# AdamClixby/Modulate

Measured on NVIDIA B200. Metric: ark_dtb_decrypt_throughput, higher is better.
Workload: dtype u8

## Files before the change

### modulate_b200/csrc/cycle_kernels.cu

```cuda
#include "cycle_kernels.cuh"
#include "lcg.h"

#include <cstdlib>

namespace modk {

using modlcg::mulmod;
using modlcg::step_lazy;
using modlcg::low8_canonical;

#ifndef MODK_CANON_FMA_MASK
#define MODK_CANON_FMA_MASK 0x5
#endif
#ifndef MODK_MIN_CTAS
#define MODK_MIN_CTAS 10
#endif
#ifndef MODK_MIN_CTAS_INLINE
#define MODK_MIN_CTAS_INLINE 8
#endif
#ifndef MODK_MIN_CTAS_COAL
#define MODK_MIN_CTAS_COAL 10
#endif
#ifndef MODK_STAGE
#define MODK_STAGE 1
#endif
#ifndef MODK_EDGE_ROUNDS
#define MODK_EDGE_ROUNDS 1
#endif
#ifndef MODK_STAGE_SEQ
#define MODK_STAGE_SEQ 1
#endif
#ifndef MODK_GENERAL_FULL
#define MODK_GENERAL_FULL 1
#endif
#ifndef MODK_HOIST_POW
#define MODK_HOIST_POW 1
#endif
#ifndef MODK_REC_PREFETCH
#define MODK_REC_PREFETCH 2048
#endif

constexpr int kTw0Size = 1024;
constexpr int kTw1Size = (int)(((1ull << 32) / kTileBytes) / kTw0Size + 2);

__constant__ uint32_t c_tw0[kTw0Size];
__constant__ uint32_t c_tw1[kTw1Size];
__constant__ uint32_t c_ainv[16];
__device__ uint32_t g_chunk_pow2[kChunksPerTile];

__device__ __forceinline__ uint32_t jump_lazy(uint32_t st, uint32_t y2)
{
    const uint64_t p = (uint64_t)st * (uint64_t)y2;
    return (uint32_t)(p >> 32) + ((uint32_t)p >> 1);
}


__device__ __forceinline__ uint4 ldg128(uint64_t addr)
{
    uint4 r;
    asm volatile("ld.global.v4.u32 {%0, %1, %2, %3}, [%4];" : "=r"(r.x), "=r"(r.y), "=r"(r.z), "=r"(r.w) : "l"(addr));
    return r;
}

__device__ __forceinline__ void stg128(uint64_t addr, const uint4& v)
{
    asm volatile("st.global.v4.u32 [%0], {%1, %2, %3, %4};" ::"l"(addr), "r"(v.x), "r"(v.y), "r"(v.z), "r"(v.w));
}

#if MODK_STAGE

__device__ __forceinline__ uint32_t smem_u32(const void* p) { return (uint32_t)__cvta_generic_to_shared(p); }

__device__ __forceinline__ void mbar_init(uint32_t bar, uint32_t count)
{
    asm volatile("mbarrier.init.shared::cta.b64 [%0], %1;" ::"r"(bar), "r"(count));
    asm volatile("fence.mbarrier_init.release.cluster;" ::: "memory");
}

__device__ __forceinline__ void mbar_expect_tx(uint32_t bar, uint32_t bytes)
{
    asm volatile("mbarrier.arrive.expect_tx.shared::cta.b64 _, [%0], %1;" ::"r"(bar), "r"(bytes) : "memory");
}

__device__ __forceinline__ void mbar_wait(uint32_t bar, uint32_t parity)
{
    asm volatile(
        "{\n"
        ".reg .pred p;\n"
        "MODK_WAIT:\n"
        "mbarrier.try_wait.parity.shared::cta.b64 p, [%0], %1;\n"
        "@p bra MODK_DONE;\n"
        "bra MODK_WAIT;\n"
        "MODK_DONE:\n"
        "}\n" ::"r"(bar), "r"(parity) : "memory");
}

__device__ __forceinline__ void bulk_g2s(uint32_t dst_smem, uint64_t src_gmem, uint32_t bytes, uint32_t bar)
{
    asm volatile("cp.async.bulk.shared::cluster.global.mbarrier::complete_tx::bytes [%0], [%1], %2, [%3];" ::"r"(dst_smem),
                 "l"(src_gmem), "r"(bytes), "r"(bar)
                 : "memory");
}

__device__ __forceinline__ uint4 lds128(uint32_t addr)
{
    uint4 r;
    asm volatile("ld.shared.v4.u32 {%0, %1, %2, %3}, [%4];" : "=r"(r.x), "=r"(r.y), "=r"(r.z), "=r"(r.w) : "r"(addr));
    return r;
}
#endif


__device__ __forceinline__ uint32_t low8_canonical_fma(uint32_t s, uint32_t two)
{
    uint32_t r;
    asm("mad.hi.u32 %0, %1, %2, %1;" : "=r"(r) : "r"(s), "r"(two));
    return r;
}

__device__ __noinline__ uint4 cycle_chunk_exact(uint4 d, uint32_t s, const uint32_t two)
{
    uint32_t w[4] = {d.x, d.y, d.z, d.w};
#pragma unroll
    for (int j = 0; j < 4; ++j) {
        s = step_lazy(s);
        const uint32_t b0 = (MODK_CANON_FMA_MASK & 1) ? low8_canonical_fma(s, two) : low8_canonical(s);
        s = step_lazy(s);
        const uint32_t b1 = (MODK_CANON_FMA_MASK & 2) ? low8_canonical_fma(s, two) : low8_canonical(s);
        s = step_lazy(s);
        const uint32_t b2 = (MODK_CANON_FMA_MASK & 4) ? low8_canonical_fma(s, two) : low8_canonical(s);
        s = step_lazy(s);
        const uint32_t b3 = (MODK_CANON_FMA_MASK & 8) ? low8_canonical_fma(s, two) : low8_canonical(s);
        const uint32_t lo = __byte_perm(b0, b1, 0x0040);
        const uint32_t hi = __byte_perm(b2, b3, 0x0040);
        w[j] ^= __byte_perm(lo, hi, 0x5410);
    }
    return make_uint4(w[0], w[1], w[2], w[3]);
}


__device__ __noinline__ void store_partial(uint64_t addr, uint4 v, uint32_t lo, uint32_t hi)
{
    const uint32_t w[4] = {v.x, v.y, v.z, v.w};
#pragma unroll
    for (uint32_t k = 0; k < 4; ++k) {
        const uint32_t b0 = 4u * k;
        if (lo <= b0 && b0 + 4u <= hi) {
            asm volatile("st.global.u32 [%0], %1;" ::"l"(addr + b0), "r"(w[k]));
        } else {
#pragma unroll
            for (uint32_t b = b0; b < b0 + 4u; ++b)
                if (b >= lo && b < hi)
                    asm volatile("st.global.u8 [%0], %1;" ::"l"(addr + b), "r"((w[k] >> (8u * (b - b0))) & 0xFFu));
        }
    }
}

__device__ __noinline__ void slow_chunk(uint64_t src_byte0, uint64_t dst_chunk, uint32_t lo, uint32_t hi, uint32_t s,
                                        uint32_t two)
{
    uint32_t w[4] = {0u, 0u, 0u, 0u};
#pragma unroll
    for (uint32_t b = 0; b < 16; ++b) {
        if (b >= lo && b < hi) {
            uint32_t byte;
            asm volatile("ld.global.u8 %0, [%1];" : "=r"(byte) : "l"(src_byte0 + b));
            w[b >> 2] |= byte << (8u * (b & 3u));
        }
    }
    store_partial(dst_chunk, cycle_chunk_exact(make_uint4(w[0], w[1], w[2], w[3]), s, two), lo, hi);
}


template <int kWs, int U, bool kStaged, bool kFull = false>
__device__ __forceinline__ void process_tile(const uint64_t src_tile, const uint64_t dst_tile, const uint32_t st,
                                             const uint32_t n_valid, const uint32_t head, const uint32_t tail,
                                             const uint32_t bs, const uint32_t idx0, const uint32_t (&pw)[U],
                                             const uint32_t two, const uint32_t stage, const uint32_t bar)
{
    constexpr uint32_t T = (uint32_t)kThreadsPerCta;
    uint4 own[U], nxt[U];
    const uint64_t sp = src_tile + 16ull * idx0;
    if (!kStaged) {
#pragma unroll
        for (int u = 0; u < U; ++u) {
            own[u] = make_uint4(0u, 0u, 0u, 0u);
            nxt[u] = make_uint4(0u, 0u, 0u, 0u);
            if (kFull || idx0 + (uint32_t)u * T < n_valid) {
                own[u] = ldg128(sp + 16ull * T * u);
                if (kWs >= 0)
                    nxt[u] = ldg128(sp + 16ull * T * u + 16ull);
            }
        }
    }

    uint32_t s[U];
#pragma unroll
    for (int u = 0; u < U; ++u)
        s[u] = jump_lazy(st, pw[u]);

    uint32_t ks[U][4];
    uint32_t any = 0u;
#if !defined(MODK_EXPERIMENT_COPY_ONLY)
#pragma unroll
    for (int j = 0; j < 4; ++j) {
#pragma unroll
        for (int u = 0; u < U; ++u) {
            const uint32_t b0 = step_lazy(s[u]);
            const uint32_t b1 = step_lazy(b0);
            const uint32_t b2 = step_lazy(b1);
            const uint32_t b3 = step_lazy(b2);
            s[u] = b3;
            const uint32_t lo = __byte_perm(b0, b1, 0x7340);
            const uint32_t hi = __byte_perm(b2, b3, 0x7340);
            any |= lo | hi;
            ks[u][j] = __byte_perm(lo, hi, 0x5410);
        }
    }
#else
#pragma unroll
    for (int u = 0; u < U; ++u)
        ks[u][0] = ks[u][1] = ks[u][2] = ks[u][3] = s[u] & two;
#endif
    const bool redo = (any & 0x80800000u) != 0u;

#if MODK_STAGE
    auto load_staged = [&](const int u) {
        own[u] = make_uint4(0u, 0u, 0u, 0u);
        nxt[u] = make_uint4(0u, 0u, 0u, 0u);
        if (kFull || idx0 + (uint32_t)u * T < n_valid) {
            own[u] = lds128(stage + 16u * (idx0 + (uint32_t)u * T));
            if (kWs >= 0)
                nxt[u] = lds128(stage + 16u * (idx0 + (uint32_t)u * T) + 16u);
        }
    };
    if (kStaged) {
        mbar_wait(bar, 0u);
#if !MODK_STAGE_SEQ
#pragma unroll
        for (int u = 0; u < U; ++u)
            load_staged(u);
#endif
    }
#else
    auto load_staged = [&](const int) {};
#endif

    const uint32_t f_lo = head ? 1u : 0u;
    const uint32_t f_hi = max(n_valid - (tail < 16u ? 1u : 0u), f_lo);
    const uint64_t dp = dst_tile + 16ull * idx0;
    auto source = [&](const int u) {
        uint4 data = own[u];
        if (kWs >= 0) {
            const uint32_t w[8] = {own[u].x, own[u].y, own[u].z, own[u].w, nxt[u].x, nxt[u].y, nxt[u].z, nxt[u].w};
            constexpr int k = kWs < 0 ? 0 : kWs;
            data.x = __funnelshift_r(w[k + 0], w[k + 1], bs);
            data.y = __funnelshift_r(w[k + 1], w[k + 2], bs);
            data.z = __funnelshift_r(w[k + 2], w[k + 3], bs);
            data.w = __funnelshift_r(w[k + 3], w[k + 4], bs);
        }
        return data;
    };
    auto emit = [&](const int u, const uint4& out) {
        const uint32_t idx = idx0 + (uint32_t)u * T;
        if (kFull || idx - f_lo < f_hi - f_lo)
            stg128(dp + 16ull * T * u, out);
        else if (idx < n_valid)
            store_partial(dp + 16ull * T * u, out, idx == 0u ? head : 0u, idx + 1u == n_valid ? tail : 16u);
    };
    if (__builtin_expect(redo, 0)) {
#if MODK_STAGE_SEQ
        if (kStaged) {
#pragma unroll
            for (int u = 0; u < U; ++u)
                load_staged(u);
        }
#endif
#pragma unroll 1
        for (int u = 0; u < U; ++u) {
            const uint32_t idx = idx0 + (uint32_t)u * T;
            uint4 data = own[0];
#pragma unroll
            for (int v = 0; v < U; ++v)
                if (v == u)
                    data = source(v);
            const uint4 out = cycle_chunk_exact(data, jump_lazy(st, __ldg(&g_chunk_pow2[idx])), two);
#pragma unroll
            for (int v = 0; v < U; ++v)
                if (v == u)
                    emit(v, out);
        }
        return;
    }
#pragma unroll
    for (int u = 0; u < U; ++u) {
#if MODK_STAGE_SEQ
        if (kStaged)
            load_staged(u);
#endif
        const uint4 data = source(u);
        emit(u, make_uint4(data.x ^ ks[u][0], data.y ^ ks[u][1], data.z ^ ks[u][2], data.w ^ ks[u][3]));
    }
}

template <int U, bool kGeneral>
__device__ __forceinline__ void run_tile(const BatchArgs& a, const int64_t src_rel, const int64_t dst_rel,
                                         const uint32_t st, const uint32_t geom, const uint32_t idx0,
                                         const uint32_t (&pw)[U], const uint32_t stage, const uint32_t bar)
{
    const uint64_t dst_tile = (uint64_t)a.dst + (uint64_t)dst_rel;
    const uint64_t sv = (uint64_t)a.src + (uint64_t)src_rel;
    const uint32_t shift = (uint32_t)sv & 15u;
    const uint64_t src_tile = sv - shift;
    constexpr uint32_t kFullGeom = (uint32_t)kChunksPerTile | (16u << 16);
    if (!kGeneral && geom == kFullGeom && shift == 0u && src_tile >= a.src_lo16 && src_tile + kTileBytes <= a.src_hi16) {
        process_tile<-1, U, false, true>(src_tile, dst_tile, st, (uint32_t)kChunksPerTile, 0u, 16u, 0u, idx0, pw, a.two, stage, bar);
        return;
    }
    const uint32_t n_valid = geom & 0xFFFu, head = (geom >> 12) & 15u, tail = (geom >> 16) & 31u;

    const uint64_t src_end = src_tile + 16ull * (n_valid + (shift ? 1u : 0u));
    if (__builtin_expect(src_tile < a.src_lo16 || src_end > a.src_hi16 || (!kGeneral && shift != 0u), 0)) {
#pragma unroll 1
        for (int u = 0; u < U; ++u) {
            const uint32_t idx = idx0 + (uint32_t)u * (uint32_t)kThreadsPerCta;
            if (idx < n_valid)
                slow_chunk(sv + 16ull * idx, dst_tile + 16ull * idx, idx == 0u ? head : 0u,
                           idx + 1u == n_valid ? tail : 16u, jump_lazy(st, g_chunk_pow2[idx]), a.two);
        }
        return;
    }

    const uint32_t bs = (shift & 3u) * 8u;
    if (!kGeneral) {
#if MODK_EDGE_ROUNDS
        if (U == 4 && n_valid <= 3u * (uint32_t)kThreadsPerCta) {
            if (n_valid <= (uint32_t)kThreadsPerCta) {
                const uint32_t p1[1] = {pw[0]};
                process_tile<-1, 1, false, false>(src_tile, dst_tile, st, n_valid, head, tail, bs, idx0, p1, a.two, stage, bar);
            } else if (n_valid <= 2u * (uint32_t)kThreadsPerCta) {
                const uint32_t p2[2] = {pw[0], pw[1]};
                process_tile<-1, 2, false, false>(src_tile, dst_tile, st, n_valid, head, tail, bs, idx0, p2, a.two, stage, bar);
            } else {
                const uint32_t p3[3] = {pw[0], pw[1], pw[2]};
                process_tile<-1, 3, false, false>(src_tile, dst_tile, st, n_valid, head, tail, bs, idx0, p3, a.two, stage, bar);
            }
            return;
        }
#endif
        process_tile<-1, U, false, false>(src_tile, dst_tile, st, n_valid, head, tail, bs, idx0, pw, a.two, stage, bar);
        return;
    }
    constexpr bool kStaged = MODK_STAGE != 0;
#if MODK_STAGE
    if (threadIdx.x == 0) {
        const uint32_t bytes = 16u * (n_valid + (shift ? 1u : 0u));
        mbar_expect_tx(bar, bytes);
        bulk_g2s(stage, src_tile, bytes, bar);
    }
#endif
#if MODK_GENERAL_FULL
    if (geom == kFullGeom) {
        switch (shift ? (int)(shift >> 2) : -1) {
        case -1: process_tile<-1, U, kStaged, true>(src_tile, dst_tile, st, n_valid, head, tail, bs, idx0, pw, a.two, stage, bar); break;
        case 0: process_tile<0, U, kStaged, true>(src_tile, dst_tile, st, n_valid, head, tail, bs, idx0, pw, a.two, stage, bar); break;
        case 1: process_tile<1, U, kStaged, true>(src_tile, dst_tile, st, n_valid, head, tail, bs, idx0, pw, a.two, stage, bar); break;
        case 2: process_tile<2, U, kStaged, true>(src_tile, dst_tile, st, n_valid, head, tail, bs, idx0, pw, a.two, stage, bar); break;
        default: process_tile<3, U, kStaged, true>(src_tile, dst_tile, st, n_valid, head, tail, bs, idx0, pw, a.two, stage, bar); break;
        }
        return;
    }
#endif
    if (shift == 0u) {
        process_tile<-1, U, kStaged>(src_tile, dst_tile, st, n_valid, head, tail, bs, idx0, pw, a.two, stage, bar);
    } else {
        switch (shift >> 2) {
        case 0: process_tile<0, U, kStaged>(src_tile, dst_tile, st, n_valid, head, tail, bs, idx0, pw, a.two, stage, bar); break;
        case 1: process_tile<1, U, kStaged>(src_tile, dst_tile, st, n_valid, head, tail, bs, idx0, pw, a.two, stage, bar); break;
        case 2: process_tile<2, U, kStaged>(src_tile, dst_tile, st, n_valid, head, tail, bs, idx0, pw, a.two, stage, bar); break;
        default: process_tile<3, U, kStaged>(src_tile, dst_tile, st, n_valid, head, tail, bs, idx0, pw, a.two, stage, bar); break;
        }
    }
}

__device__ __forceinline__ uint32_t tile_start_state(uint32_t n0, uint32_t h0, uint32_t tin)
{
    const uint32_t st = mulmod(n0, c_ainv[h0]);
    return mulmod(st, mulmod(c_tw0[tin & (uint32_t)(kTw0Size - 1)], c_tw1[tin / (uint32_t)kTw0Size]));
}

__device__ __forceinline__ TileRec make_tile_rec(uint64_t src_off, uint64_t dst_off, uint32_t len, uint32_t n0,
                                                 uint32_t tin, uint32_t dst_align, uint32_t entry)
{
    const uint32_t h0 = (dst_align + (uint32_t)dst_off) & 15u;
    const uint64_t span = (uint64_t)h0 + len;
    const uint32_t nchunks = (uint32_t)((span + 15u) >> 4);
    const uint32_t c_begin = tin * (uint32_t)kChunksPerTile;
    const uint32_t n_valid = min((uint32_t)kChunksPerTile, nchunks - c_begin);
    const bool last = c_begin + n_valid == nchunks;
    TileRec r;
    r.src_rel = (int64_t)src_off - (int64_t)h0 + 16ll * (int64_t)c_begin;
    r.dst_rel = (int64_t)dst_off - (int64_t)h0 + 16ll * (int64_t)c_begin;
    r.state = tile_start_state(n0, h0, tin);
    r.geom = pack_geom(n_valid, tin == 0u ? h0 : 0u, last ? (((uint32_t)span - 1u) & 15u) + 1u : 16u);
    r.entry = entry;
    r.pad = 0u;
    return r;
}

#if MODK_STAGE
#define MODK_STAGE_SETUP                                                                          \
    uint32_t stage = 0u, bar = 0u;                                                                \
    if (kGeneral) {                                                                               \
        __shared__ __align__(128) uint8_t s_stage[kTileBytes + 16];                               \
        __shared__ __align__(8) uint64_t s_bar;                                                   \
        stage = smem_u32(s_stage);                                                                \
        bar = smem_u32(&s_bar);                                                                   \
        if (threadIdx.x == 0)                                                                     \
            mbar_init(bar, 1u);                                                                   \
        __syncthreads();                                                                          \
    }
#else
#define MODK_STAGE_SETUP const uint32_t stage = 0u, bar = 0u;
#endif

template <int U>
__device__ __forceinline__ void load_chunk_pows(uint32_t (&pw)[U], uint32_t idx0)
{
#pragma unroll
    for (int u = 0; u < U; ++u)
        pw[u] = __ldg(&g_chunk_pow2[idx0 + (uint32_t)u * (uint32_t)kThreadsPerCta]);
}

template <bool kGeneral>
__global__ void __launch_bounds__(kThreadsPerCta, kGeneral ? MODK_MIN_CTAS : MODK_MIN_CTAS_COAL)
cycle_batch_kernel(const BatchArgs a)
{
    MODK_STAGE_SETUP
    const uint4* p = reinterpret_cast<const uint4*>(a.tiles + blockIdx.x);
    uint32_t pw[kUnroll];
#if MODK_HOIST_POW
    load_chunk_pows<kUnroll>(pw, threadIdx.x);
#endif
    const uint4 lo = __ldg(p);
    const uint4 hi = __ldg(p + 1);
#if MODK_REC_PREFETCH
    if (threadIdx.x == 0 && a.n_tiles - blockIdx.x > (uint32_t)MODK_REC_PREFETCH) {
        const uint64_t ahead = (uint64_t)(a.tiles + blockIdx.x + MODK_REC_PREFETCH);
        if ((ahead & 127u) == 0u)
            asm volatile("prefetch.global.L2 [%0];" ::"l"(ahead));
    }
#endif
    const int64_t src_rel = (int64_t)((uint64_t)lo.x | ((uint64_t)lo.y << 32));
    const int64_t dst_rel = (int64_t)((uint64_t)lo.z | ((uint64_t)lo.w << 32));
#if !MODK_HOIST_POW
    load_chunk_pows<kUnroll>(pw, threadIdx.x);
#endif
    run_tile<kUnroll, kGeneral>(a, src_rel, dst_rel, hi.x, hi.y, threadIdx.x, pw, stage, bar);
}

template <bool kGeneral>
__global__ void __launch_bounds__(kThreadsPerCta, kGeneral ? MODK_MIN_CTAS_INLINE : MODK_MIN_CTAS_COAL)
cycle_inline_kernel(const BatchArgs a, const __grid_constant__ InlineDescs in)
{
    MODK_STAGE_SETUP
    uint32_t pw[kUnroll];
    load_chunk_pows<kUnroll>(pw, threadIdx.x);
    const uint32_t tile = blockIdx.x;
    const uint32_t e = tile / a.tiles_per_entry;
    const DevDesc& d = in.d[e];
    const TileRec r = make_tile_rec(d.src_off, d.dst_off, d.len, d.neg_state, tile - d.first_tile,
                                    (uint32_t)(uintptr_t)a.dst & 15u, e);
    run_tile<kUnroll, kGeneral>(a, r.src_rel, r.dst_rel, r.state, r.geom, threadIdx.x, pw, stage, bar);
}

__global__ void build_tiles_kernel(const DevDesc* __restrict__ descs, uint32_t n_descs, uint32_t dst_align,
                                   TileRec* __restrict__ tiles, uint32_t n_tiles)
{
    const uint32_t t = blockIdx.x * blockDim.x + threadIdx.x;
    if (t >= n_tiles)
        return;
    uint32_t lo = 0, hi = n_descs;
    while (hi - lo > 1) {
        const uint32_t mid = lo + ((hi - lo) >> 1);
        if (descs[mid].first_tile <= t)
            lo = mid;
        else
            hi = mid;
    }
    const DevDesc d = descs[lo];
    tiles[t] = make_tile_rec(d.src_off, d.dst_off, d.len, d.neg_state, t - d.first_tile, dst_align, lo);
}


cudaError_t upload_tables()
{
    static uint32_t h_tw0[kTw0Size], h_tw1[kTw1Size], h_ainv[16], h_chunk[kChunksPerTile];
    static const bool built = []() {
        for (int j = 0; j < kTw0Size; ++j)
            h_tw0[j] = modlcg::pow_a((uint64_t)kTileBytes * (uint64_t)j);
        for (int j = 0; j < kTw1Size; ++j)
            h_tw1[j] = modlcg::pow_a((uint64_t)kTileBytes * (uint64_t)kTw0Size * (uint64_t)j);
        for (int h = 0; h < 16; ++h)
            h_ainv[h] = modlcg::pow_a_inv((uint64_t)h);
        for (int j = 0; j < kChunksPerTile; ++j)
            h_chunk[j] = 2u * modlcg::pow_a(16ull * (uint64_t)j);
        return true;
    }();
    (void)built;
    cudaError_t err;
    if ((err = cudaMemcpyToSymbol(c_tw0, h_tw0, sizeof(h_tw0))) != cudaSuccess) return err;
    if ((err = cudaMemcpyToSymbol(c_tw1, h_tw1, sizeof(h_tw1))) != cudaSuccess) return err;
    if ((err = cudaMemcpyToSymbol(c_ainv, h_ainv, sizeof(h_ainv))) != cudaSuccess) return err;
    if ((err = cudaMemcpyToSymbol(g_chunk_pow2, h_chunk, sizeof(h_chunk))) != cudaSuccess) return err;
    return cudaSuccess;
}

constexpr uint32_t kMaxGrid = 0x7FFFFFFFu;

static bool coaligned(const BatchArgs& a)
{
    if (a.uniform_delta < 0 || getenv("MOD_FORCE_GENERAL") != nullptr)
        return false;
    return (((uintptr_t)a.src - (uintptr_t)a.dst + (uintptr_t)a.uniform_delta) & 15u) == 0u;
}

cudaError_t launch_batch(const BatchArgs& args, cudaStream_t stream)
{
    for (uint32_t t0 = 0; t0 < args.n_tiles;) {
        const uint32_t n = args.n_tiles - t0 < kMaxGrid ? args.n_tiles - t0 : kMaxGrid;
        BatchArgs a = args;
        a.tiles = args.tiles + t0;
        a.n_tiles = n;
        if (coaligned(args))
            cycle_batch_kernel<false><<<n, kThreadsPerCta, 0, stream>>>(a);
        else
            cycle_batch_kernel<true><<<n, kThreadsPerCta, 0, stream>>>(a);
        const cudaError_t err = cudaGetLastError();
        if (err != cudaSuccess)
            return err;
        t0 += n;
    }
    return cudaSuccess;
}

cudaError_t launch_batch_inline(const BatchArgs& args, const InlineDescs& descs, cudaStream_t stream)
{
    if (args.n_tiles == 0)
        return cudaSuccess;
    if (coaligned(args))
        cycle_inline_kernel<false><<<args.n_tiles, kThreadsPerCta, 0, stream>>>(args, descs);
    else
        cycle_inline_kernel<true><<<args.n_tiles, kThreadsPerCta, 0, stream>>>(args, descs);
    return cudaGetLastError();
}

cudaError_t launch_build_tiles(const DevDesc* descs, uint32_t n_descs, uint32_t dst_align, TileRec* tiles,
                               uint32_t n_tiles, cudaStream_t stream)
{
    if (n_tiles == 0)
        return cudaSuccess;
    const unsigned threads = 256;
    build_tiles_kernel<<<(n_tiles + threads - 1) / threads, threads, 0, stream>>>(descs, n_descs, dst_align,
                                                                                 tiles, n_tiles);
    return cudaGetLastError();
}

}
```

Before: 3483.

## Write full coalesced tiles via shared memory and bulk async copy to global

For full aligned tiles in the coalesced kernel, each thread now writes its output chunks to a shared-memory staging buffer. One thread then issues a cp.async.bulk shared-to-global copy of the whole tile. This is meant to replace many per-thread 128-bit global stores with a single bulk transfer. In exchange it adds a __syncthreads and a blocking wait_group per tile, which serialises work, and the extra shared memory may reduce occupancy.

```diff
diff --git a/modulate_b200/csrc/cycle_kernels.cu b/modulate_b200/csrc/cycle_kernels.cu
--- a/modulate_b200/csrc/cycle_kernels.cu
+++ b/modulate_b200/csrc/cycle_kernels.cu
@@ -38,6 +38,9 @@
 #endif
 #ifndef MODK_REC_PREFETCH
 #define MODK_REC_PREFETCH 2048
+#endif
+#ifndef MODK_BULK_STORE
+#define MODK_BULK_STORE 1
 #endif
 
 constexpr int kTw0Size = 1024;
@@ -67,9 +70,28 @@
     asm volatile("st.global.v4.u32 [%0], {%1, %2, %3, %4};" ::"l"(addr), "r"(v.x), "r"(v.y), "r"(v.z), "r"(v.w));
 }
 
+__device__ __forceinline__ uint32_t smem_u32(const void* p) { return (uint32_t)__cvta_generic_to_shared(p); }
+
+#if MODK_BULK_STORE
+__device__ __forceinline__ void sts128(uint32_t addr, const uint4& v)
+{
+    asm volatile("st.shared.v4.u32 [%0], {%1, %2, %3, %4};" ::"r"(addr), "r"(v.x), "r"(v.y), "r"(v.z), "r"(v.w) : "memory");
+}
+
+__device__ __forceinline__ void bulk_store_tile(uint64_t dst_gmem, uint32_t src_smem, uint32_t bytes)
+{
+    asm volatile("fence.proxy.async.shared::cta;" ::: "memory");
+    __syncthreads();
+    if (threadIdx.x == 0) {
+        asm volatile("cp.async.bulk.global.shared::cta.bulk_group [%0], [%1], %2;" ::"l"(dst_gmem), "r"(src_smem), "r"(bytes)
+                     : "memory");
+        asm volatile("cp.async.bulk.commit_group;" ::: "memory");
+        asm volatile("cp.async.bulk.wait_group.read 0;" ::: "memory");
+    }
+}
+#endif
+
 #if MODK_STAGE
-
-__device__ __forceinline__ uint32_t smem_u32(const void* p) { return (uint32_t)__cvta_generic_to_shared(p); }
 
 __device__ __forceinline__ void mbar_init(uint32_t bar, uint32_t count)
 {
@@ -172,7 +194,7 @@
 }
 
 
-template <int kWs, int U, bool kStaged, bool kFull = false>
+template <int kWs, int U, bool kStaged, bool kFull = false, bool kBulkOut = false>
 __device__ __forceinline__ void process_tile(const uint64_t src_tile, const uint64_t dst_tile, const uint32_t st,
                                              const uint32_t n_valid, const uint32_t head, const uint32_t tail,
                                              const uint32_t bs, const uint32_t idx0, const uint32_t (&pw)[U],
@@ -261,8 +283,14 @@
         }
         return data;
     };
+    static_assert(!kBulkOut || (kFull && !kStaged), "bulk stores are for whole tiles whose stage holds no source");
     auto emit = [&](const int u, const uint4& out) {
         const uint32_t idx = idx0 + (uint32_t)u * T;
+#if MODK_BULK_STORE
+        if (kBulkOut)
+            sts128(stage + 16u * idx, out);
+        else
+#endif
         if (kFull || idx - f_lo < f_hi - f_lo)
             stg128(dp + 16ull * T * u, out);
         else if (idx < n_valid)
@@ -290,17 +318,21 @@
                 if (v == u)
                     emit(v, out);
         }
-        return;
-    }
-#pragma unroll
-    for (int u = 0; u < U; ++u) {
+    } else {
+#pragma unroll
+        for (int u = 0; u < U; ++u) {
 #if MODK_STAGE_SEQ
-        if (kStaged)
-            load_staged(u);
-#endif
-        const uint4 data = source(u);
-        emit(u, make_uint4(data.x ^ ks[u][0], data.y ^ ks[u][1], data.z ^ ks[u][2], data.w ^ ks[u][3]));
-    }
+            if (kStaged)
+                load_staged(u);
+#endif
+            const uint4 data = source(u);
+            emit(u, make_uint4(data.x ^ ks[u][0], data.y ^ ks[u][1], data.z ^ ks[u][2], data.w ^ ks[u][3]));
+        }
+    }
+#if MODK_BULK_STORE
+    if (kBulkOut)
+        bulk_store_tile(dst_tile, stage, kTileBytes);
+#endif
 }
 
 template <int U, bool kGeneral>
@@ -314,7 +346,8 @@
     const uint64_t src_tile = sv - shift;
     constexpr uint32_t kFullGeom = (uint32_t)kChunksPerTile | (16u << 16);
     if (!kGeneral && geom == kFullGeom && shift == 0u && src_tile >= a.src_lo16 && src_tile + kTileBytes <= a.src_hi16) {
-        process_tile<-1, U, false, true>(src_tile, dst_tile, st, (uint32_t)kChunksPerTile, 0u, 16u, 0u, idx0, pw, a.two, stage, bar);
+        process_tile<-1, U, false, true, MODK_BULK_STORE != 0>(src_tile, dst_tile, st, (uint32_t)kChunksPerTile, 0u, 16u, 0u,
+                                                               idx0, pw, a.two, stage, bar);
         return;
     }
     const uint32_t n_valid = geom & 0xFFFu, head = (geom >> 12) & 15u, tail = (geom >> 16) & 31u;
@@ -408,6 +441,16 @@
     return r;
 }
 
+#if MODK_BULK_STORE
+#define MODK_BULK_STORE_SETUP                                                                     \
+    if (!kGeneral) {                                                                              \
+        __shared__ __align__(128) uint8_t s_out[kTileBytes];                                      \
+        stage = smem_u32(s_out);                                                                  \
+    }
+#else
+#define MODK_BULK_STORE_SETUP
+#endif
+
 #if MODK_STAGE
 #define MODK_STAGE_SETUP                                                                          \
     uint32_t stage = 0u, bar = 0u;                                                                \
@@ -419,9 +462,10 @@
         if (threadIdx.x == 0)                                                                     \
             mbar_init(bar, 1u);                                                                   \
         __syncthreads();                                                                          \
-    }
+    }                                                                                             \
+    MODK_BULK_STORE_SETUP
 #else
-#define MODK_STAGE_SETUP const uint32_t stage = 0u, bar = 0u;
+#define MODK_STAGE_SETUP uint32_t stage = 0u; const uint32_t bar = 0u; MODK_BULK_STORE_SETUP
 #endif
 
 template <int U>
```

Result: no change. 3507 (median of 6 runs) (+0.7%).
